# sparisi/pvr_habitat

Measured on AMD Instinct MI355X. Metric: frames/sec embedded (ResNet50, 256x256), higher is better.
Workload: dtype f16; 1 GPU; configs[1]: ResNet50 (MoCo-v2 layout) frozen, 256x256 uint8 frames resident in HBM, batch 256/GPU, random-init synthetic weights, f16 storage / MFMA inputs with fp32 accumulation (the product default, inside the 1e-3 parity bound; configs[1] names bf16); global_batch=256, frame=256, chunk=256, batches_in_flight=2, parallelism=frame shards, no collective (dp1)

## Files before the change

pvr_habitat_amd/csrc/bottleneck_chain.hip:

```cpp
#include "encoder_internal.h"

namespace pvr {


__device__ __forceinline__ void ch_dma16(__amdgpu_buffer_rsrc_t rs, char *lds, int voff, int soff) {
    __builtin_amdgcn_raw_ptr_buffer_load_lds(rs, (__attribute__((address_space(3))) void *)lds, 16, voff, soff, 0, 0);
}

#ifdef CHAIN_STAMP
__device__ unsigned long long chain_stamps[8192][12];
#define CH_T(i_) { if (threadIdx.x == 0) ch_tt[i_] = __builtin_amdgcn_s_memrealtime(); }
#else
#define CH_T(i_)
#endif

#ifndef CH_KNOCK
#define CH_KNOCK 0
#endif
template <int AUX = 0>
__device__ __forceinline__ void store_b128_imm(u32x4 v, __amdgpu_buffer_rsrc_t rs, int voff, int imm) {
    if constexpr (!(CH_KNOCK & 1)) __builtin_amdgcn_raw_buffer_store_b128(v, rs, voff + imm, 0, AUX);
}

template <int CM, int CMN, bool F16, int RD, int OCC, bool HALO, bool DS = false, int PFK = -1>
__global__ __launch_bounds__(256, OCC) void bottleneck_chain_kernel(ChainP p) {
    typedef typename HT<F16>::V8 V8;
    constexpr int BM = 128, BK = 64, BN = CM;
    constexpr int A_CH = BM / 32, B_CH = BN / 32, TM = 4, TN = BN / 32;
    constexpr int KS = CM / 64, HROWS = CM == 64 ? 256 : 192, RL = CM == 64 ? 3 : 2;
    constexpr int HSL = HROWS * 128, RING_OFF = KS * HSL, SLICE = CM * 128, ZERO_OFF = (HROWS - 1) * 128;
    constexpr int HOPS = KS * HROWS / 32;
    constexpr int STAGE = HALO ? (RING_OFF + 2 * SLICE) / 2 : (BM + BN) * 128;
    constexpr int C4 = 4 * CM, G = C4 / 64, KS3 = CM / 64;
    constexpr int TN1 = CMN / 32;
    constexpr int W3_CH = CM / 32, W1_CH = CMN / 32;
    constexpr int T2_OFF = 0;
    constexpr int YG_OFF = KS3 * 16384;
    constexpr int W3_OFF = YG_OFF + 16384;
    constexpr int W1_OFF = W3_OFF + KS3 * 8192;
    static_assert(W3_OFF + KS3 * 8192 <= 2 * STAGE, "phase-B tiles must fit the phase-A area");
    static_assert(RD >= 1 && RD <= G, "residual prefetch depth");
    extern __shared__ __attribute__((aligned(16))) char smem[];

    const int tid = threadIdx.x, lane = tid & 63, wave = tid >> 6;
#ifdef CHAIN_STAMP
    unsigned long long ch_tt[12] = {0, 0, 0, 0, 0, 0, 0, 0, 0, 0, 0, 0};
#endif
    CH_T(0);
    const int m0 = xcd_remap(blockIdx.x, gridDim.x) * BM;
    const int srow = tid >> 3, pch = tid & 7;
    const auto rs_in = __builtin_amdgcn_make_buffer_rsrc(const_cast<u16 *>(p.in), 0, p.in_bytes, 0x00020000);
    const auto rs_w2 = __builtin_amdgcn_make_buffer_rsrc(const_cast<u16 *>(p.w2), 0, p.w2_bytes, 0x00020000);
    const auto rs_w3 = __builtin_amdgcn_make_buffer_rsrc(const_cast<u16 *>(p.w3), 0, p.w3_bytes, 0x00020000);
    const auto rs_w1 = __builtin_amdgcn_make_buffer_rsrc(const_cast<u16 *>(p.w1n), 0, p.w1n_bytes, 0x00020000);
    const auto rs_res = __builtin_amdgcn_make_buffer_rsrc(const_cast<u16 *>(DS ? p.xds : p.res), 0, DS ? p.xds_bytes : p.y_bytes, 0x00020000);
    const auto rs_wd = __builtin_amdgcn_make_buffer_rsrc(const_cast<u16 *>(DS ? p.wds : p.w3), 0, DS ? p.wds_bytes : p.w3_bytes, 0x00020000);
    const auto rs_y = __builtin_amdgcn_make_buffer_rsrc(p.y, 0, p.y_bytes, 0x00020000);
    const auto rs_t = __builtin_amdgcn_make_buffer_rsrc(p.t1n, 0, p.t1n_bytes, 0x00020000);
    constexpr int OOB = 0x7ffffff0;

    if constexpr (HALO) {
        const int HR = 128 + 2 * p.W + 2, hbase = m0 - p.W - 1;
#pragma unroll
        for (int i = 0; i < HOPS; ++i) {
            const int o = i * 4 + wave, sl = o / (HROWS / 8), rb = o % (HROWS / 8);
            const int r = rb * 8 + (lane >> 3), c = (lane & 7) ^ (r & 6);
            const int vo = (r < HR && hbase + r >= 0) ? ((hbase + r) * CM + sl * 64 + c * 8) * 2 : OOB;
            ch_dma16(rs_in, smem + sl * HSL + rb * 1024, vo, 0);
        }
    }

    int a_off[A_CH], a_mask[A_CH];
#pragma unroll
    for (int i = 0; i < A_CH; ++i) {
        const int row = srow + 32 * i;
        const int lch = pch ^ ((row >> 1) & 7);
        const int m = m0 + row;
        const bool ok = m < p.M;
        const int mm = ok ? m : 0;
        const int wo = mm % p.Wo, t = mm / p.Wo, ho = t % p.Ho, n = t / p.Ho;
        const int hi0 = ho * p.stride - 1, wi0 = wo * p.stride - 1;
        a_off[i] = (((n * p.H + hi0) * p.W + wi0) * CM + lch * 8) * 2;
        int hb = 0, wb = 0;
#pragma unroll
        for (int t3 = 0; t3 < 3; ++t3) {
            hb |= (int)(ok && (unsigned)(hi0 + t3) < (unsigned)p.H) << t3;
            wb |= (int)((unsigned)(wi0 + t3) < (unsigned)p.W) << t3;
        }
        int mask = 0;
#pragma unroll
        for (int t3 = 0; t3 < 3; ++t3) mask |= ((hb >> t3) & 1) ? (wb << (t3 * 3)) : 0;
        a_mask[i] = mask;
    }
    int b_off[B_CH];
#pragma unroll
    for (int i = 0; i < B_CH; ++i) {
        const int row = srow + 32 * i;
        b_off[i] = (row * (9 * CM) + (pch ^ ((row >> 1) & 7)) * 8) * 2;
    }
    const int lds_st = srow * 128 + pch * 16;
    u32x4 ra[A_CH], rb[B_CH];
    constexpr int cpt = CM / BK, nk = 9 * cpt;
    int kh = 0, kw = 0, cs = 0, tap = 0;
#define PVR_LOAD_SLICE(kt_)                                                                             \
    {                                                                                                   \
        const int tap_off = ((kh * p.W + kw) * CM + cs * BK) * 2;                                       \
        _Pragma("unroll") for (int i = 0; i < A_CH; ++i) {                                              \
            const int vo = ((a_mask[i] >> tap) & 1) ? a_off[i] + tap_off : OOB;                         \
            ra[i] = __builtin_bit_cast(u32x4, __builtin_amdgcn_raw_buffer_load_b128(rs_in, vo, 0, 0));  \
        }                                                                                               \
        _Pragma("unroll") for (int i = 0; i < B_CH; ++i)                                                \
            rb[i] = __builtin_bit_cast(u32x4, __builtin_amdgcn_raw_buffer_load_b128(rs_w2, b_off[i], (kt_) * (BK * 2), 0)); \
        if (++cs == cpt) { cs = 0; ++tap; if (++kw == 3) { kw = 0; ++kh; } }                            \
    }
#define PVR_STORE_SLICE(buf_)                                                                           \
    {                                                                                                   \
        char *base = smem + (buf_) * STAGE + lds_st;                                                    \
        _Pragma("unroll") for (int i = 0; i < A_CH; ++i)                                                \
            *reinterpret_cast<u32x4 *>(base + i * 32 * 128) = ra[i];                                    \
        _Pragma("unroll") for (int i = 0; i < B_CH; ++i)                                                \
            *reinterpret_cast<u32x4 *>(base + BM * 128 + i * 32 * 128) = rb[i];                         \
    }

    const int wm = wave >> 1, wn = wave & 1;
    const int fr = lane & 15, fq = lane >> 4;
    int x_rd[2][TM];
    int b_rd[2][TN];
#pragma unroll
    for (int ks = 0; ks < 2; ++ks) {
#pragma unroll
        for (int j = 0; j < TM; ++j) {
            const int row = wm * 64 + j * 16 + fr;
            x_rd[ks][j] = row * 128 + (((ks * 4 + fq) ^ ((row >> 1) & 7)) << 4);
        }
#pragma unroll
        for (int i = 0; i < TN; ++i) {
            const int row = wn * (BN / 2) + i * 16 + fr;
            b_rd[ks][i] = BM * 128 + row * 128 + (((ks * 4 + fq) ^ ((row >> 1) & 7)) << 4);
        }
    }

    const int y_nhwc = ((m0 + wm * 64 + fr) * C4 + wn * 32 + fq * 8) * 2;
    const int y_blkd = ((m0 >> 4) + wm * 4) * (C4 * 32) + (wn * 4 + fq) * 256 + fr * 16;
    const int y_off0 = p.y_blk ? y_blkd : y_nhwc, y_js = p.y_blk ? C4 * 32 : 16 * C4 * 2, y_gs = p.y_blk ? 2048 : 128;
    const int r_off0 = p.res_blk ? y_blkd : y_nhwc, r_js = p.res_blk ? C4 * 32 : 16 * C4 * 2, r_gs = p.res_blk ? 2048 : 128;
    const int t_nhwc = ((m0 + wm * 64 + fr) * CMN + wn * (CMN / 2) + fq * 8) * 2;
    const int t_blkd = ((m0 >> 4) + wm * 4) * (CMN * 32) + (wn * (CMN / 16) + fq) * 256 + fr * 16;
    const int t_off0 = p.t_blk ? t_blkd : t_nhwc, t_js = p.t_blk ? CMN * 32 : 16 * CMN * 2;
#define Y_OFF(j_) (y_off0 + (j_) * y_js)
#define R_OFF(j_) (r_off0 + (j_) * r_js)
#define T_OFF(j_) (t_off0 + (j_) * t_js)
    const int st_r = tid >> 3, st_c = ((tid & 7) ^ ((st_r >> 1) & 7)) * 16;
    const int w3_g0 = st_r * CM * 2 + st_c, w3_l0 = W3_OFF + st_r * 128 + (tid & 7) * 16;
    const int w1_g0 = st_r * C4 * 2 + st_c, w1_l0 = W1_OFF + st_r * 128 + (tid & 7) * 16;
#define W3_G(i_) (w3_g0 + ((i_) & 1) * (32 * CM * 2) + ((i_) >> 1) * 128)
#define W3_L(i_) (w3_l0 + ((i_) & 1) * 4096 + ((i_) >> 1) * 8192)
#define W1_G(i_) (w1_g0 + (i_) * (32 * C4 * 2))
#define W1_L(i_) (w1_l0 + (i_) * 4096)
    u32x4 rres[RD][TM], w3r[W3_CH], w1r[CMN ? W1_CH : 1];
#define PVR_PHASE_B_PREFETCH()                                                                                          \
    {                                                                                                                   \
        if constexpr (!DS) {                                                                                            \
            _Pragma("unroll") for (int d = 0; d < RD; ++d)                                                              \
                _Pragma("unroll") for (int j = 0; j < TM; ++j)                                                          \
                    rres[d][j] = __builtin_bit_cast(u32x4, __builtin_amdgcn_raw_buffer_load_b128(rs_res, (CH_KNOCK & 2) ? OOB : R_OFF(j), d * r_gs, DS ? 0 : PVR_NT_AUX(16))); \
        }                                                                                                               \
        _Pragma("unroll") for (int i = 0; i < W3_CH; ++i)                                                               \
            w3r[i] = __builtin_bit_cast(u32x4, __builtin_amdgcn_raw_buffer_load_b128(rs_w3, W3_G(i), 0, 0));            \
        if constexpr (CMN > 0) {                                                                                        \
            _Pragma("unroll") for (int i = 0; i < W1_CH; ++i)                                                           \
                w1r[i] = __builtin_bit_cast(u32x4, __builtin_amdgcn_raw_buffer_load_b128(rs_w1, W1_G(i), 0, 0));        \
        }                                                                                                               \
    }
    if constexpr (!HALO || PFK < 0) PVR_PHASE_B_PREFETCH();

    f32x4 acc2[TN][TM];
#pragma unroll
    for (int i = 0; i < TN; ++i)
#pragma unroll
        for (int j = 0; j < TM; ++j) acc2[i][j] = f32x4{0.f, 0.f, 0.f, 0.f};
    if constexpr (HALO) {
        u32x4 w2r[RL][B_CH];
#pragma unroll
        for (int q = 0; q < RL; ++q)
#pragma unroll
            for (int i = 0; i < B_CH; ++i)
                w2r[q][i] = __builtin_bit_cast(u32x4, __builtin_amdgcn_raw_buffer_load_b128(rs_w2, b_off[i], q * (BK * 2), 0));
        asm volatile("s_waitcnt vmcnt(0)" ::: "memory");
#pragma unroll
        for (int i = 0; i < B_CH; ++i) *reinterpret_cast<u32x4 *>(smem + RING_OFF + lds_st + i * 32 * 128) = w2r[0][i];
        __syncthreads();
        CH_T(1);
        int h_row[TM], h_mask[TM];
#pragma unroll
        for (int j = 0; j < TM; ++j) {
            const int pr = wm * 64 + j * 16 + fr, m = m0 + pr;
            const bool ok = m < p.M;
            const int mm = ok ? m : 0;
            const int wo = mm % p.W, ho = (mm / p.W) % p.H;
            int hb = 0, wb_ = 0;
#pragma unroll
            for (int t3 = 0; t3 < 3; ++t3) {
                hb |= (int)(ok && (unsigned)(ho - 1 + t3) < (unsigned)p.H) << t3;
                wb_ |= (int)((unsigned)(wo - 1 + t3) < (unsigned)p.W) << t3;
            }
            int mask = 0;
#pragma unroll
            for (int t3 = 0; t3 < 3; ++t3) mask |= ((hb >> t3) & 1) ? (wb_ << (t3 * 3)) : 0;
            h_row[j] = pr; h_mask[j] = mask;
        }
#pragma unroll
        for (int kt = 0; kt < nk; ++kt) {
            if (kt == PFK) PVR_PHASE_B_PREFETCH();
            if (kt + RL < nk) {
#pragma unroll
                for (int i = 0; i < B_CH; ++i)
                    w2r[kt % RL][i] = __builtin_bit_cast(u32x4, __builtin_amdgcn_raw_buffer_load_b128(rs_w2, (CH_KNOCK & 8) ? OOB : b_off[i], (kt + RL) * (BK * 2), 0));
            }
            const int tp = kt / KS, csl = kt % KS, shift = (tp / 3) * p.W + tp % 3;
            int xo[TM];
#pragma unroll
            for (int j = 0; j < TM; ++j) {
                const int r = h_row[j] + shift;
                const int a = csl * HSL + r * 128 + ((fq ^ (r & 6)) << 4);
                xo[j] = ((h_mask[j] >> tp) & 1) ? a : ZERO_OFF;
            }
            const char *ring = smem + RING_OFF + (kt & 1) * SLICE - BM * 128;
#pragma unroll
            for (int ks = 0; ks < 2; ++ks) {
                V8 xa[TM], wb[TN];
#pragma unroll
                for (int j = 0; j < TM; ++j) if constexpr (!(CH_KNOCK & 32)) xa[j] = *reinterpret_cast<const V8 *>(smem + (xo[j] ^ (ks * 64)));
#pragma unroll
                for (int i = 0; i < TN; ++i) if constexpr (!(CH_KNOCK & 32)) wb[i] = *reinterpret_cast<const V8 *>(ring + b_rd[ks][i]);
#pragma unroll
                for (int i = 0; i < TN; ++i)
#pragma unroll
                    for (int j = 0; j < TM; ++j) acc2[i][j] = mfma16<F16>(wb[i], xa[j], acc2[i][j]);
            }
            if (kt + 1 < nk) {
#pragma unroll
                for (int i = 0; i < B_CH; ++i)
                    if constexpr (!(CH_KNOCK & 4)) *reinterpret_cast<u32x4 *>(smem + RING_OFF + ((kt + 1) & 1) * SLICE + lds_st + i * 32 * 128) = w2r[(kt + 1) % RL][i];
            }
            if constexpr (!(CH_KNOCK & 16)) __syncthreads();
        }
    } else {
    PVR_LOAD_SLICE(0);
    PVR_STORE_SLICE(0);
    __syncthreads();
    CH_T(1);
#define PVR_K_STEP(kt_, CUR_)                                                                           \
    {                                                                                                   \
        const bool more = (kt_) + 1 < nk;                                                               \
        if (more) PVR_LOAD_SLICE((kt_) + 1);                                                            \
        const char *sb = smem + (CUR_) * STAGE;                                                         \
        _Pragma("unroll") for (int ks = 0; ks < 2; ++ks) {                                              \
            V8 xa[TM], wb[TN];                                                                          \
            _Pragma("unroll") for (int j = 0; j < TM; ++j) xa[j] = *reinterpret_cast<const V8 *>(sb + x_rd[ks][j]); \
            _Pragma("unroll") for (int i = 0; i < TN; ++i) wb[i] = *reinterpret_cast<const V8 *>(sb + b_rd[ks][i]); \
            _Pragma("unroll") for (int i = 0; i < TN; ++i)                                              \
                _Pragma("unroll") for (int j = 0; j < TM; ++j) acc2[i][j] = mfma16<F16>(wb[i], xa[j], acc2[i][j]); \
        }                                                                                               \
        if (more) PVR_STORE_SLICE(1 - (CUR_));                                                          \
        __syncthreads();                                                                                \
    }
    for (int kt = 0; kt < nk; kt += 2) {
        PVR_K_STEP(kt, 0);
        if (kt + 1 < nk) PVR_K_STEP(kt + 1, 1);
    }
    }
    CH_T(2);
    V8 xd[2][TM], wdr[2][2];
    int wd_off[2];
    if constexpr (DS) {
#pragma unroll
        for (int j = 0; j < TM; ++j) {
            const int xo_ = (m0 + wm * 64 + j * 16 + fr) * 128 + fq * 16;
#pragma unroll
            for (int ks = 0; ks < 2; ++ks) xd[ks][j] = __builtin_bit_cast(V8, __builtin_amdgcn_raw_buffer_load_b128(rs_res, xo_, ks * 64, 0));
        }
#pragma unroll
        for (int t = 0; t < 2; ++t) {
            wd_off[t] = (wn * 32 + t * 16 + fr) * 128 + fq * 16;
#pragma unroll
            for (int ks = 0; ks < 2; ++ks) wdr[t][ks] = __builtin_bit_cast(V8, __builtin_amdgcn_raw_buffer_load_b128(rs_wd, wd_off[t] + ks * 64, 0, 0));
        }
    }
#undef PVR_K_STEP
#undef PVR_LOAD_SLICE
#undef PVR_STORE_SLICE

#pragma unroll
    for (int i = 0; i < TN; ++i) {
        const int c = wn * (BN / 2) + i * 16 + fq * 4;
        const float4 bv = *reinterpret_cast<const float4 *>(p.b2 + c);
#pragma unroll
        for (int j = 0; j < TM; ++j) {
            const int row = wm * 64 + j * 16 + fr;
            const f32x4 a = acc2[i][j];
            const unsigned lo = pack2_h<F16>(fmaxf(a[0] + bv.x, 0.f), fmaxf(a[1] + bv.y, 0.f));
            const unsigned hi = pack2_h<F16>(fmaxf(a[2] + bv.z, 0.f), fmaxf(a[3] + bv.w, 0.f));
            const int cc = c & 63;
            char *dst = smem + T2_OFF + (c >> 6) * 16384 + row * 128 + ((((cc >> 3) ^ ((row >> 1) & 7))) << 4) + (cc & 4) * 2;
            *reinterpret_cast<uint2 *>(dst) = make_uint2(lo, hi);
        }
    }
#pragma unroll
    for (int i = 0; i < W3_CH; ++i) *reinterpret_cast<u32x4 *>(smem + W3_L(i)) = w3r[i];
    if constexpr (CMN > 0) {
#pragma unroll
        for (int i = 0; i < W1_CH; ++i) *reinterpret_cast<u32x4 *>(smem + W1_L(i)) = w1r[i];
    }
    if (G > 1) {
#pragma unroll
        for (int i = 0; i < W3_CH; ++i)
            w3r[i] = __builtin_bit_cast(u32x4, __builtin_amdgcn_raw_buffer_load_b128(rs_w3, W3_G(i), 64 * CM * 2, 0));
        if constexpr (CMN > 0) {
#pragma unroll
            for (int i = 0; i < W1_CH; ++i) w1r[i] = __builtin_bit_cast(u32x4, __builtin_amdgcn_raw_buffer_load_b128(rs_w1, W1_G(i), 128, 0));
        }
    }
    __syncthreads();
    CH_T(3);

    int w3_rd[2][2], w1_rd[2][CMN ? TN1 : 1], yg_wr[TM];
#pragma unroll
    for (int ks = 0; ks < 2; ++ks) {
#pragma unroll
        for (int t = 0; t < 2; ++t) {
            const int row = wn * 32 + t * 16 + fr;
            w3_rd[ks][t] = W3_OFF + row * 128 + (((ks * 4 + fq) ^ ((row >> 1) & 7)) << 4);
        }
        if constexpr (CMN > 0) {
#pragma unroll
            for (int i = 0; i < TN1; ++i) {
                const int row = wn * (CMN / 2) + i * 16 + fr;
                w1_rd[ks][i] = W1_OFF + row * 128 + (((ks * 4 + fq) ^ ((row >> 1) & 7)) << 4);
            }
        }
    }
#pragma unroll
    for (int j = 0; j < TM; ++j) {
        const int row = wm * 64 + j * 16 + fr;
        yg_wr[j] = YG_OFF + row * 128 + (((wn * 4 + fq) ^ ((row >> 1) & 7)) << 4);
    }
    f32x4 acc1[CMN ? TN1 : 1][TM];
    if constexpr (CMN > 0) {
#pragma unroll
        for (int i = 0; i < TN1; ++i)
#pragma unroll
            for (int j = 0; j < TM; ++j) acc1[i][j] = f32x4{0.f, 0.f, 0.f, 0.f};
    }

#pragma unroll
    for (int g = 0; g < G; ++g) {
        if (g == 1) CH_T(6);
        f32x4 acc3[2][TM];
#pragma unroll
        for (int t = 0; t < 2; ++t)
#pragma unroll
            for (int j = 0; j < TM; ++j) acc3[t][j] = f32x4{0.f, 0.f, 0.f, 0.f};
#pragma unroll
        for (int s = 0; s < KS3; ++s)
#pragma unroll
            for (int ks = 0; ks < 2; ++ks) {
                V8 xa[TM], wb[2];
#pragma unroll
                for (int j = 0; j < TM; ++j) xa[j] = *reinterpret_cast<const V8 *>(smem + T2_OFF + s * 16384 + x_rd[ks][j]);
#pragma unroll
                for (int t = 0; t < 2; ++t) wb[t] = *reinterpret_cast<const V8 *>(smem + s * 8192 + w3_rd[ks][t]);
#pragma unroll
                for (int t = 0; t < 2; ++t)
#pragma unroll
                    for (int j = 0; j < TM; ++j) acc3[t][j] = mfma16<F16>(wb[t], xa[j], acc3[t][j]);
            }
        if constexpr (DS) {
#pragma unroll
            for (int ks = 0; ks < 2; ++ks)
#pragma unroll
                for (int t = 0; t < 2; ++t)
#pragma unroll
                    for (int j = 0; j < TM; ++j) acc3[t][j] = mfma16<F16>(wdr[t][ks], xd[ks][j], acc3[t][j]);
            if (g + 1 < G) {
#pragma unroll
                for (int t = 0; t < 2; ++t)
#pragma unroll
                    for (int ks = 0; ks < 2; ++ks)
                        wdr[t][ks] = __builtin_bit_cast(V8, __builtin_amdgcn_raw_buffer_load_b128(rs_wd, wd_off[t] + ks * 64, (g + 1) * 8192, 0));
            }
        }
        if (g == 1) CH_T(7);
        const int c0 = g * 64 + wn * 32 + fq * 8;
        const float4 bA = *reinterpret_cast<const float4 *>(p.b3 + c0), bB = *reinterpret_cast<const float4 *>(p.b3 + c0 + 4);
#pragma unroll
        for (int j = 0; j < TM; ++j) {
            const f32x4 lo = acc3[0][j], hi = acc3[1][j];
            float v[8] = {lo[0] + bA.x, lo[1] + bA.y, lo[2] + bA.z, lo[3] + bA.w, hi[0] + bB.x, hi[1] + bB.y, hi[2] + bB.z, hi[3] + bB.w};
            u32x4 o;
            if constexpr (DS) {
#pragma unroll
                for (int e = 0; e < 4; ++e)
                    o[e] = pack2_h<F16>(fmaxf(v[2 * e], 0.f), fmaxf(v[2 * e + 1], 0.f));
            } else {
                const u32x4 r = rres[g % RD][j];
#pragma unroll
                for (int e = 0; e < 4; ++e) {
                    const float v0 = fmaxf(v[2 * e] + from_h<F16>((u16)(r[e] & 0xffffu)), 0.f);
                    const float v1 = fmaxf(v[2 * e + 1] + from_h<F16>((u16)(r[e] >> 16)), 0.f);
                    o[e] = pack2_h<F16>(v0, v1);
                }
            }
            if (p.y_blk) store_b128_imm<PVR_NT_AUX(4)>(o, rs_y, Y_OFF(j) + g * y_gs, 0);
            else store_b128_imm(o, rs_y, Y_OFF(j) + g * y_gs, 0);
            if constexpr (CMN > 0) *reinterpret_cast<u32x4 *>(smem + yg_wr[j]) = o;
        }
        if (!DS && g + RD < G) {
#pragma unroll
            for (int j = 0; j < TM; ++j)
                rres[g % RD][j] = __builtin_bit_cast(u32x4, __builtin_amdgcn_raw_buffer_load_b128(rs_res, (CH_KNOCK & 2) ? OOB : R_OFF(j), (g + RD) * r_gs, DS ? 0 : PVR_NT_AUX(16)));
        }
        if (g == 1) CH_T(8);
        __syncthreads();
        if (g == 1) CH_T(9);
        if (g + 1 < G) {
#pragma unroll
            for (int i = 0; i < W3_CH; ++i) *reinterpret_cast<u32x4 *>(smem + W3_L(i)) = w3r[i];
            if (g + 2 < G) {
#pragma unroll
                for (int i = 0; i < W3_CH; ++i)
                    w3r[i] = __builtin_bit_cast(u32x4, __builtin_amdgcn_raw_buffer_load_b128(rs_w3, W3_G(i), (g + 2) * (64 * CM * 2), 0));
            }
        }
        if (g == 1) CH_T(10);
        if constexpr (CMN == 0) __syncthreads();
        if constexpr (CMN > 0) {
#pragma unroll
            for (int ks = 0; ks < 2; ++ks) {
                V8 xa[TM], wb[TN1];
#pragma unroll
                for (int j = 0; j < TM; ++j) xa[j] = *reinterpret_cast<const V8 *>(smem + YG_OFF + x_rd[ks][j]);
#pragma unroll
                for (int i = 0; i < TN1; ++i) wb[i] = *reinterpret_cast<const V8 *>(smem + w1_rd[ks][i]);
#pragma unroll
                for (int i = 0; i < TN1; ++i)
#pragma unroll
                    for (int j = 0; j < TM; ++j) acc1[i][j] = mfma16<F16>(wb[i], xa[j], acc1[i][j]);
            }
            __syncthreads();
            if (g == 1) CH_T(11);
            if (g + 1 < G) {
#pragma unroll
                for (int i = 0; i < W1_CH; ++i) *reinterpret_cast<u32x4 *>(smem + W1_L(i)) = w1r[i];
                if (g + 2 < G) {
#pragma unroll
                    for (int i = 0; i < W1_CH; ++i)
                        w1r[i] = __builtin_bit_cast(u32x4, __builtin_amdgcn_raw_buffer_load_b128(rs_w1, W1_G(i), (g + 2) * 128, 0));
                }
            }
        }
    }

    CH_T(4);
    if constexpr (CMN > 0) {
#pragma unroll
        for (int q = 0; q < TN1 / 2; ++q) {
            const int c0 = wn * (CMN / 2) + q * 32 + fq * 8;
            const float4 bA = *reinterpret_cast<const float4 *>(p.b1n + c0), bB = *reinterpret_cast<const float4 *>(p.b1n + c0 + 4);
#pragma unroll
            for (int j = 0; j < TM; ++j) {
                const f32x4 lo = acc1[2 * q][j], hi = acc1[2 * q + 1][j];
                const float v[8] = {lo[0] + bA.x, lo[1] + bA.y, lo[2] + bA.z, lo[3] + bA.w, hi[0] + bB.x, hi[1] + bB.y, hi[2] + bB.z, hi[3] + bB.w};
                u32x4 o;
#pragma unroll
                for (int e = 0; e < 4; ++e)
                    o[e] = pack2_h<F16>(fmaxf(v[2 * e], 0.f), fmaxf(v[2 * e + 1], 0.f));
                if (p.t_blk) store_b128_imm<0>(o, rs_t, T_OFF(j) + q * 1024, 0);
                else store_b128_imm<PVR_NT_AUX(8)>(o, rs_t, T_OFF(j), q * 64);
            }
        }
    }
#undef PVR_PHASE_B_PREFETCH
#undef W3_G
#undef W3_L
#undef W1_G
#undef W1_L
#undef Y_OFF
#undef R_OFF
#undef T_OFF
#ifdef CHAIN_STAMP
    CH_T(5);
    if (threadIdx.x == 0 && blockIdx.x < 8192) { _Pragma("unroll") for (int k = 0; k < 12; ++k) chain_stamps[blockIdx.x][k] = ch_tt[k]; }
#endif
}

template <int CM, int CMN, bool F16, int RD, int OCC, bool HALO, bool DS = false, int PFK = -1>
static pvr_status launch_chain_one(ChainP &p, hipStream_t stream) {
    const int grid = (p.M + 127) / 128;
    const size_t pipe = HALO ? (size_t)(CM / 64) * (CM == 64 ? 256 : 192) * 128 + (size_t)2 * CM * 128 : (size_t)2 * (128 + CM) * 128;
    const size_t phase_b = (CM / 64) * 16384 + 16384 + (CM / 64) * 8192 + CMN * 128;
    const size_t lds = phase_b <= pipe ? pipe : phase_b;
    static DeviceOnce attr_done;
    if (attr_done.needed()) {
        PVR_HIP_TRY(hipFuncSetAttribute((const void *)bottleneck_chain_kernel<CM, CMN, F16, RD, OCC, HALO, DS, PFK>,
                                        hipFuncAttributeMaxDynamicSharedMemorySize, (int)lds));
        attr_done.mark();
    }
    hipLaunchKernelGGL((bottleneck_chain_kernel<CM, CMN, F16, RD, OCC, HALO, DS, PFK>), dim3(grid), dim3(256), lds, stream, p);
    PVR_LAUNCH_CHECK();
    return PVR_OK;
}

template <int CM, int CMN, bool F16, int RD, int OCC, bool DS = false>
static pvr_status launch_chain_inst(ChainP &p, const PlanSwitches &sw, hipStream_t stream) {
    const bool halo = p.stride == 1 && 128 + 2 * p.W + 2 <= (CM == 64 ? 256 : 192) - 1 && sw.chain_halo;
    if constexpr (DS) {
        if (halo) return sw.chain_ds_occ == 3 ? launch_chain_one<CM, CMN, F16, RD, 3, true, true>(p, stream) : launch_chain_one<CM, CMN, F16, RD, 2, true, true>(p, stream);
        return launch_chain_one<CM, CMN, F16, RD, 2, false, true>(p, stream);
    } else {
        if (halo) {
            if constexpr (CM == 128) {
                if (sw.chain_pfk == 12) return launch_chain_one<CM, CMN, F16, RD, 2, true, false, 12>(p, stream);
            }
            return launch_chain_one<CM, CMN, F16, RD, (CM == 64 ? OCC : 2), true>(p, stream);
        }
        return launch_chain_one<CM, CMN, F16, RD, OCC, false>(p, stream);
    }
}

template <bool F16>
static pvr_status launch_chain_dt(ChainP &p, int cm, int cmn, const PlanSwitches &sw, hipStream_t stream) {
    if (p.xds) {
        if (cm == 64 && cmn == 64) return launch_chain_inst<64, 64, F16, 1, 2, true>(p, sw, stream);
        set_error("bottleneck chain with downsample: no instance for Cm=%d, next Cm=%d", cm, cmn);
        return PVR_ERR_INVALID;
    }
    const int cfg = sw.chain_cfg;
#define PVR_CHAIN64(CMN_)                                                                 \
    switch (cfg) {                                                                        \
    case 12: return launch_chain_inst<64, CMN_, F16, 1, 2>(p, sw, stream);                \
    case 13: return launch_chain_inst<64, CMN_, F16, 1, 3>(p, sw, stream);                \
    case 22: return launch_chain_inst<64, CMN_, F16, 2, 2>(p, sw, stream);                \
    case 23: return launch_chain_inst<64, CMN_, F16, 2, 3>(p, sw, stream);                \
    default: return launch_chain_inst<64, CMN_, F16, 4, 2>(p, sw, stream);                \
    }
    if (cm == 64 && cmn == 64) PVR_CHAIN64(64)
    if (cm == 64 && cmn == 128) {
        if (cfg / 10 == 1) return launch_chain_inst<64, 128, F16, 1, 2>(p, sw, stream);
        if (cfg / 10 == 2) return launch_chain_inst<64, 128, F16, 2, 2>(p, sw, stream);
        return launch_chain_inst<64, 128, F16, 4, 2>(p, sw, stream);
    }
    if (cm == 64 && cmn == 0) PVR_CHAIN64(0)
#undef PVR_CHAIN64
    if (cm == 128 && cmn == 128) return launch_chain_inst<128, 128, F16, 1, 2>(p, sw, stream);
    if (cm == 128 && cmn == 0) return launch_chain_inst<128, 0, F16, 1, 2>(p, sw, stream);
    set_error("bottleneck chain: no instance for Cm=%d, next Cm=%d", cm, cmn);
    return PVR_ERR_INVALID;
}

bool chain_uses_wave_form(const PlanSwitches &sw, int cm, int cmn, int stride, bool ds) { return sw.chain_wave && chain_wave_supported(sw, cm, cmn, stride, ds); }

bool chain_uses_wave128(const PlanSwitches &sw, int cm, int cmn, int stride, int64_t M) { return sw.chain_wave && chain_wave128_supported(sw, cm, cmn, stride, M); }

bool chain_ds_supported(int cm, int cmn, int cin, int stride) { return cm == 64 && cmn == 64 && cin == 64 && stride == 1; }
bool chain_supported(int cm, int cmn) { return (cm == 64 && (cmn == 0 || cmn == 64 || cmn == 128)) || (cm == 128 && (cmn == 0 || cmn == 128)); }

int chain_row_source(int row) { return (row & ~31) + 8 * ((row >> 2) & 3) + 4 * ((row >> 4) & 1) + (row & 3); }

pvr_status launch_bottleneck_chain(const PlanSwitches &sw, const void *t1, const void *w2, const float *b2, const void *w3p, const float *b3, const void *res,
                                   void *y, const void *w1np, const float *b1n, void *t1n, int n, int h, int w, int cm, int cmn,
                                   int stride, int dtype, hipStream_t stream, const void *xds, const void *wdsp, const void *w3pb, const void *wdspb,
                                   int wave, int in_blk, int out_blk, const void *wpk, int y_s2) {
    PVR_REQUIRE(chain_supported(cm, cmn), "bottleneck chain: unsupported widths Cm=%d next=%d", cm, cmn);
    PVR_REQUIRE(t1 && w2 && b2 && w3p && b3 && (res || xds) && y && (cmn == 0 || (w1np && b1n && t1n)), "bottleneck chain: null argument");
    PVR_REQUIRE(!xds || (wdsp && chain_ds_supported(cm, cmn, 64, stride)), "bottleneck chain with downsample: unsupported shape");
    ChainP p;
    p.in = (const u16 *)t1; p.w2 = (const u16 *)w2; p.w3 = (const u16 *)w3p; p.w1n = (const u16 *)w1np; p.res = (const u16 *)res;
    p.b2 = b2; p.b3 = b3; p.b1n = b1n; p.y = (u16 *)y; p.t1n = (u16 *)t1n;
    p.N = n; p.H = h; p.W = w; p.stride = stride;
    p.Ho = (h + 2 - 3) / stride + 1; p.Wo = (w + 2 - 3) / stride + 1;
    const int64_t M = (int64_t)n * p.Ho * p.Wo;
    const int64_t inb = (int64_t)n * h * w * cm * 2, yb = M * 4 * cm * 2, tb = M * (cmn ? cmn : 1) * 2;
    PVR_REQUIRE(inb < 0x7ffffff0ll && yb < 0x7ffffff0ll && tb < 0x7ffffff0ll, "bottleneck chain: operand larger than 2 GiB (use a smaller chunk)");
    p.M = (int)M; p.in_bytes = (unsigned)inb; p.y_bytes = (unsigned)yb; p.t1n_bytes = (unsigned)tb;
    p.xds = (const u16 *)xds; p.wds = (const u16 *)wdsp;
    p.xds_bytes = xds ? (unsigned)(M * 64 * 2) : 0; p.wds_bytes = xds ? (unsigned)(4 * cm * 64 * 2) : 0;
    p.w2_bytes = (unsigned)(cm * 9 * cm * 2); p.w3_bytes = (unsigned)(4 * cm * cm * 2); p.w1n_bytes = (unsigned)(cmn * 4 * cm * 2);
    if (wave == 2) {
        PVR_REQUIRE(chain_wave128_supported(sw, cm, cmn, stride, M) && !xds, "bottleneck chain: no layer2 wave form for Cm=%d next=%d stride=%d", cm, cmn, stride);
        p.wpk = (const u16 *)wpk; p.in_blk = in_blk; p.out_blk = out_blk & 1;
        return launch_chain_wave128(p, cmn, dtype, stream);
    }
    if (wave) {
        PVR_REQUIRE(chain_wave_supported(sw, cm, cmn, stride, xds != nullptr), "bottleneck chain: no wave form for Cm=%d next=%d stride=%d", cm, cmn, stride);
        p.w3b = (const u16 *)w3pb; p.wdsb = (const u16 *)wdspb; p.in_blk = in_blk; p.out_blk = out_blk; p.y_s2 = y_s2;
        return launch_chain_wave(p, cmn, sw.chain_wave_halo, dtype, stream);
    }
    PVR_REQUIRE(!y_s2, "bottleneck chain: y_s2 is a store of the wave form");
    PVR_REQUIRE(!(in_blk || out_blk) || M % 16 == 0, "bottleneck chain: the blocked layout needs a multiple of 16 pixels");
    p.res_blk = xds ? 0 : in_blk; p.y_blk = out_blk & 1;
    p.t_blk = (out_blk & 2) && cmn > 0;
    return dtype == PVR_F16 ? launch_chain_dt<true>(p, cm, cmn, sw, stream) : launch_chain_dt<false>(p, cm, cmn, sw, stream);
}

}
```

Baseline: 103,700 frames/s.

## Hand-schedule CM=128 bottleneck chain 3x3 and conv3 loops with explicit LDS double-buffering

For the CM=128 halo path with prefetch, the 3x3 conv main loop is replaced by a hand-scheduled version. It DMAs w2 slices straight into LDS with buffer_load_lds, issues inline-asm ds_read_b128 into two fragment sets, and uses explicit lgkmcnt waits and sched_barriers so the next fragment loads overlap the current MFMA set. The conv3 loop for CM=128 is similarly unrolled into four stages with software-pipelined LDS reads. The aim is to hide LDS latency behind MFMAs, which the compiler's own schedule did not do. The cost is fragile inline asm, tighter register pressure, and a wait-count scheme that assumes issue order is kept.

```diff
diff --git a/pvr_habitat_amd/csrc/bottleneck_chain.hip b/pvr_habitat_amd/csrc/bottleneck_chain.hip
--- a/pvr_habitat_amd/csrc/bottleneck_chain.hip
+++ b/pvr_habitat_amd/csrc/bottleneck_chain.hip
@@ -40,6 +40,7 @@
     constexpr int W1_OFF = W3_OFF + KS3 * 8192;
     static_assert(W3_OFF + KS3 * 8192 <= 2 * STAGE, "phase-B tiles must fit the phase-A area");
     static_assert(RD >= 1 && RD <= G, "residual prefetch depth");
+    constexpr bool PIPE3 = CM == 128 && !(HALO && PFK < 0);
     extern __shared__ __attribute__((aligned(16))) char smem[];
 
     const int tid = threadIdx.x, lane = tid & 63, wave = tid >> 6;
@@ -174,12 +175,106 @@
     }
     if constexpr (!HALO || PFK < 0) PVR_PHASE_B_PREFETCH();
 
+#define CH_RD(dst_, addr_) asm volatile("ds_read_b128 %0, %1" : "=v"(dst_) : "v"(addr_))
+#define CH_WAIT8(n_, X_, W_)                                                                                            \
+    asm volatile("s_waitcnt lgkmcnt(" #n_ ")" : "+v"(X_[0]), "+v"(X_[1]), "+v"(X_[2]), "+v"(X_[3]), "+v"(W_[0]), "+v"(W_[1]), "+v"(W_[2]), "+v"(W_[3]))
+#define CH_WAIT6(n_, X_, W_)                                                                                            \
+    asm volatile("s_waitcnt lgkmcnt(" #n_ ")" : "+v"(X_[0]), "+v"(X_[1]), "+v"(X_[2]), "+v"(X_[3]), "+v"(W_[0]), "+v"(W_[1]))
+
     f32x4 acc2[TN][TM];
 #pragma unroll
     for (int i = 0; i < TN; ++i)
 #pragma unroll
         for (int j = 0; j < TM; ++j) acc2[i][j] = f32x4{0.f, 0.f, 0.f, 0.f};
-    if constexpr (HALO) {
+    if constexpr (HALO && CM == 128 && PFK >= 0) {
+        static_assert(CM != 128 || (TM == 4 && TN == 4 && KS == 2 && B_CH == 4), "hand-scheduled phase A: 4 x 4 MFMA tiles per wave");
+        const int w2_row = wave * 8 + (lane >> 3);
+        const int w2_vo = (w2_row * (9 * CM) + (((lane & 7) ^ ((w2_row >> 1) & 7)) * 8)) * 2;
+#define CH_W2_DMA(kt_)                                                                                                  \
+        _Pragma("unroll") for (int i = 0; i < 4; ++i)                                                                   \
+            ch_dma16(rs_w2, smem + RING_OFF + ((kt_) & 1) * SLICE + i * 4096 + wave * 1024, w2_vo, (kt_) * (BK * 2) + i * (32 * 9 * CM * 2));
+#define CH_MFMA_SET(s_)                                                                                                 \
+        _Pragma("unroll") for (int i = 0; i < TN; ++i)                                                                  \
+            _Pragma("unroll") for (int j = 0; j < TM; ++j) acc2[i][j] = mfma16<F16>(fw[s_][i], fx[s_][j], acc2[i][j]);
+        CH_W2_DMA(0);
+        asm volatile("s_waitcnt vmcnt(0)" ::: "memory");
+        __builtin_amdgcn_s_barrier();
+        __builtin_amdgcn_sched_barrier(0);
+        CH_T(1);
+        int h_row[TM], h_mask[TM];
+#pragma unroll
+        for (int j = 0; j < TM; ++j) {
+            const int pr = wm * 64 + j * 16 + fr, m = m0 + pr;
+            const bool ok = m < p.M;
+            const int mm = ok ? m : 0;
+            const int wo = mm % p.W, ho = (mm / p.W) % p.H;
+            int hb = 0, wb_ = 0;
+#pragma unroll
+            for (int t3 = 0; t3 < 3; ++t3) {
+                hb |= (int)(ok && (unsigned)(ho - 1 + t3) < (unsigned)p.H) << t3;
+                wb_ |= (int)((unsigned)(wo - 1 + t3) < (unsigned)p.W) << t3;
+            }
+            int mask = 0;
+#pragma unroll
+            for (int t3 = 0; t3 < 3; ++t3) mask |= ((hb >> t3) & 1) ? (wb_ << (t3 * 3)) : 0;
+            h_row[j] = pr; h_mask[j] = mask;
+        }
+#define CH_XO(dst_, kt_)                                                                                                \
+        {                                                                                                               \
+            const int tp_ = (kt_) / KS, csl_ = (kt_) % KS, shift_ = (tp_ / 3) * p.W + tp_ % 3;                          \
+            _Pragma("unroll") for (int j = 0; j < TM; ++j) {                                                            \
+                const int r_ = h_row[j] + shift_;                                                                       \
+                const int a_ = csl_ * HSL + r_ * 128 + ((fq ^ (r_ & 6)) << 4);                                          \
+                dst_[j] = ((h_mask[j] >> tp_) & 1) ? a_ : ZERO_OFF;                                                    \
+            }                                                                                                           \
+        }
+        V8 fx[2][TM], fw[2][TN];
+        constexpr int NPF = (DS ? 0 : RD * TM) + W3_CH + (CMN > 0 ? W1_CH : 0);
+        int xo[TM];
+        CH_XO(xo, 0);
+#pragma unroll
+        for (int j = 0; j < TM; ++j) CH_RD(fx[0][j], xo[j]);
+#pragma unroll
+        for (int kt = 0; kt < nk; ++kt) {
+            const int wbase = RING_OFF + (kt & 1) * SLICE - BM * 128;
+#pragma unroll
+            for (int i = 0; i < TN; ++i) CH_RD(fw[0][i], wbase + b_rd[0][i]);
+            if constexpr (!(CH_KNOCK & 8)) { if (kt + 1 < nk) CH_W2_DMA(kt + 1); }
+            if (kt == PFK) {
+                __builtin_amdgcn_sched_barrier(0);
+                PVR_PHASE_B_PREFETCH();
+                __builtin_amdgcn_sched_barrier(0);
+            }
+#pragma unroll
+            for (int j = 0; j < TM; ++j) CH_RD(fx[1][j], xo[j] ^ 64);
+#pragma unroll
+            for (int i = 0; i < TN; ++i) CH_RD(fw[1][i], wbase + b_rd[1][i]);
+            CH_WAIT8(8, fx[0], fw[0]);
+            __builtin_amdgcn_sched_barrier(0);
+            if (kt + 1 < nk) CH_XO(xo, kt + 1);
+            CH_MFMA_SET(0);
+            __builtin_amdgcn_sched_barrier(0);
+            if (kt + 1 < nk) {
+#pragma unroll
+                for (int j = 0; j < TM; ++j) CH_RD(fx[0][j], xo[j]);
+                CH_WAIT8(4, fx[1], fw[1]);
+            } else {
+                CH_WAIT8(0, fx[1], fw[1]);
+            }
+            __builtin_amdgcn_sched_barrier(0);
+            CH_MFMA_SET(1);
+            __builtin_amdgcn_sched_barrier(0);
+            if constexpr (!(CH_KNOCK & 64)) {
+                if (kt == PFK) asm volatile("s_waitcnt vmcnt(%0)" :: "n"(NPF) : "memory");
+                else asm volatile("s_waitcnt vmcnt(0)" ::: "memory");
+            }
+            if constexpr (!(CH_KNOCK & 16)) __builtin_amdgcn_s_barrier();
+            __builtin_amdgcn_sched_barrier(0);
+        }
+#undef CH_W2_DMA
+#undef CH_MFMA_SET
+#undef CH_XO
+    } else if constexpr (HALO) {
         u32x4 w2r[RL][B_CH];
 #pragma unroll
         for (int q = 0; q < RL; ++q)
@@ -361,6 +456,31 @@
         for (int t = 0; t < 2; ++t)
 #pragma unroll
             for (int j = 0; j < TM; ++j) acc3[t][j] = f32x4{0.f, 0.f, 0.f, 0.f};
+        if constexpr (PIPE3) {
+            static_assert(CM != 128 || (KS3 == 2 && TM == 4), "hand-scheduled conv3: four stages of 4 + 2 fragments");
+            V8 gx[2][TM], gw[2][2];
+#define CH3_READ(q_)                                                                                                    \
+            {                                                                                                           \
+                _Pragma("unroll") for (int j = 0; j < TM; ++j) CH_RD(gx[(q_) & 1][j], T2_OFF + ((q_) >> 1) * 16384 + x_rd[(q_) & 1][j]); \
+                _Pragma("unroll") for (int t = 0; t < 2; ++t) CH_RD(gw[(q_) & 1][t], ((q_) >> 1) * 8192 + w3_rd[(q_) & 1][t]); \
+            }
+#define CH3_MFMA(s_)                                                                                                    \
+            {                                                                                                           \
+                __builtin_amdgcn_sched_barrier(0);                                                                      \
+                _Pragma("unroll") for (int t = 0; t < 2; ++t)                                                           \
+                    _Pragma("unroll") for (int j = 0; j < TM; ++j) acc3[t][j] = mfma16<F16>(gw[s_][t], gx[s_][j], acc3[t][j]); \
+            }
+            CH3_READ(0); CH3_READ(1);
+            CH_WAIT6(6, gx[0], gw[0]); CH3_MFMA(0);
+            __builtin_amdgcn_sched_barrier(0);
+            CH3_READ(2); CH_WAIT6(6, gx[1], gw[1]); CH3_MFMA(1);
+            __builtin_amdgcn_sched_barrier(0);
+            CH3_READ(3); CH_WAIT6(6, gx[0], gw[0]); CH3_MFMA(0);
+            __builtin_amdgcn_sched_barrier(0);
+            CH_WAIT6(0, gx[1], gw[1]); CH3_MFMA(1);
+#undef CH3_READ
+#undef CH3_MFMA
+        } else {
 #pragma unroll
         for (int s = 0; s < KS3; ++s)
 #pragma unroll
@@ -375,6 +495,7 @@
 #pragma unroll
                     for (int j = 0; j < TM; ++j) acc3[t][j] = mfma16<F16>(wb[t], xa[j], acc3[t][j]);
             }
+        }
         if constexpr (DS) {
 #pragma unroll
             for (int ks = 0; ks < 2; ++ks)
@@ -481,6 +602,9 @@
         }
     }
 #undef PVR_PHASE_B_PREFETCH
+#undef CH_RD
+#undef CH_WAIT8
+#undef CH_WAIT6
 #undef W3_G
 #undef W3_L
 #undef W1_G
```

After: 104,200 frames/s, median of 6. About the same (+0.4%).
